# jw007123/hp-Adaptive-Signed-Distance-Field-Octree

Measured on AMD Instinct MI355X. Metric: Query() Mpts/sec at targetError=1e-5 (union3 field, 10M SplitMix64 pts per GPU, HBM-resident); Create() ms reported as create_ms, higher is better.
Workload: dtype f64

## Files before the change

hp-adaptive-signed-distance-field-octree_amd/build.py:

```python
import os
import shutil
import subprocess
import sys

HERE = os.path.dirname(os.path.abspath(__file__))
CSRC = os.path.join(HERE, "csrc")
LIBDIR = os.path.join(HERE, "lib")
LIB = os.path.join(LIBDIR, "libhpsdf.so")
HOOKS_LIB = os.path.join(LIBDIR, "libhpsdf_hooks.so")
HOOK_SOURCES = ["frontier.hip", "capi.cpp"]
INCLUDE = os.path.normpath(os.path.join(HERE, "..", "include"))

SOURCES = ["fit_mesh.hip", "fit_analytic.hip", "fit_samples.hip", "fit.hip", "kernels.hip", "mesh_field.hip", "frontier.hip", "fit_mfma.hip", "fit_low.hip", "mesh_build.hip", "cg.hip", "continuity_asm.hip", "surface.hip", "surface_sparse.hip", "query_gradient.hip", "project.hip", "tables.cpp", "builder.cpp", "mesh.cpp", "obj.cpp", "continuity.cpp", "host_query.cpp", "capi.cpp"]
HEADERS = sorted(f for f in os.listdir(CSRC) if f.endswith(".hpp"))
QUERY_SOURCES = ("kernels.hip",)
MESH_SOURCES = ("mesh_field.hip", "fit_mesh.hip")
SOURCE_GROUPS = {"query": QUERY_SOURCES, "mesh": MESH_SOURCES}
PUBLIC_HEADERS = ["hpsdf.h", "hpsdf_octree.hpp"]

FLAGS = ["-O3", "-std=c++17", "-fPIC", "-ffp-contract=off", "-fno-fast-math", "--offload-arch=gfx950",
         "-fvisibility=hidden", "-Wall", "-Wno-unused-function", "-I", INCLUDE]
FLAGS += os.environ.get("HPSDF_EXTRA_FLAGS", "").split()
FILE_FLAGS = {"fit_mfma.hip": ["-mllvm", "-amdgpu-mfma-vgpr-form=1"]}


def hipcc():
    for c in (os.environ.get("HIPCC"), "/opt/rocm/bin/hipcc", shutil.which("hipcc")):
        if c and os.path.exists(c):
            return c
    raise RuntimeError("hipcc not found: the HIP extension cannot be built (there is no CPU fallback)")


def stale():
    if not os.path.exists(LIB) or not os.path.exists(HOOKS_LIB):
        return True
    t = os.path.getmtime(LIB)
    deps = [os.path.join(CSRC, s) for s in SOURCES + HEADERS] + [os.path.join(INCLUDE, h) for h in PUBLIC_HEADERS]
    deps.append(os.path.abspath(__file__))
    return any(os.path.exists(d) and os.path.getmtime(d) > t for d in deps)


def build(force=False, verbose=False):
    if not force and not stale():
        return LIB
    os.makedirs(LIBDIR, exist_ok=True)
    objs = []
    cc = hipcc()
    objdir = os.path.join(HERE, "build")
    os.makedirs(objdir, exist_ok=True)
    procs = []
    for s in SOURCES:
        src = os.path.join(CSRC, s)
        obj = os.path.join(objdir, s + ".o")
        objs.append(obj)
        if (not force and os.path.exists(obj) and os.path.getmtime(obj) > os.path.getmtime(src)
                and all(os.path.getmtime(obj) > os.path.getmtime(os.path.join(CSRC, h)) for h in HEADERS)
                and all(os.path.getmtime(obj) > os.path.getmtime(os.path.join(INCLUDE, h)) for h in PUBLIC_HEADERS)):
            continue
        cmd = [cc] + FLAGS + FILE_FLAGS.get(s, []) + ["-c", src, "-o", obj]
        if verbose:
            print(" ".join(cmd))
        procs.append((s, subprocess.Popen(cmd, stdout=subprocess.PIPE, stderr=subprocess.STDOUT, text=True)))
    for s, p in procs:
        out, _ = p.communicate()
        if p.returncode != 0:
            raise RuntimeError("hipcc failed on %s:\n%s" % (s, out))
        if verbose and out.strip():
            print(out)
    cmd = [cc, "-shared", "-fPIC", "--offload-arch=gfx950", "-o", LIB] + objs
    r = subprocess.run(cmd, stdout=subprocess.PIPE, stderr=subprocess.STDOUT, text=True)
    if r.returncode != 0:
        raise RuntimeError("link failed:\n" + r.stdout)
    build_hooks(cc, objs, verbose)
    return LIB


def build_hooks(cc, objs, verbose=False):
    hookdir = os.path.join(HERE, "build", "hooks")
    os.makedirs(hookdir, exist_ok=True)
    procs, swapped = [], list(objs)
    for s in HOOK_SOURCES:
        obj = os.path.join(hookdir, s + ".o")
        swapped[SOURCES.index(s)] = obj
        cmd = [cc] + FLAGS + ["-DHPSDF_TEST_HOOKS"] + FILE_FLAGS.get(s, []) + ["-c", os.path.join(CSRC, s), "-o", obj]
        if verbose:
            print(" ".join(cmd))
        procs.append((s, subprocess.Popen(cmd, stdout=subprocess.PIPE, stderr=subprocess.STDOUT, text=True)))
    for s, p in procs:
        out, _ = p.communicate()
        if p.returncode != 0:
            raise RuntimeError("hipcc failed on %s (hooks):\n%s" % (s, out))
    r = subprocess.run([cc, "-shared", "-fPIC", "--offload-arch=gfx950", "-o", HOOKS_LIB] + swapped, stdout=subprocess.PIPE,
                       stderr=subprocess.STDOUT, text=True)
    if r.returncode != 0:
        raise RuntimeError("link failed (hooks):\n" + r.stdout)
    return HOOKS_LIB


LAB_LIB = os.path.join(LIBDIR, "libhpsdf_lab.so")


def build_variant(name, flags, sources=QUERY_SOURCES, verbose=False):
    lib = build()
    cc = hipcc()
    out = os.path.join(LIBDIR, "libhpsdf_%s.so" % name)
    if os.path.exists(out) and os.path.getmtime(out) > os.path.getmtime(lib):
        return out
    vdir = os.path.join(HERE, "build", "variant_" + name)
    os.makedirs(vdir, exist_ok=True)
    objs = [os.path.join(HERE, "build", s + ".o") for s in SOURCES]
    procs = []
    for s in sources:
        obj = os.path.join(vdir, s + ".o")
        objs[SOURCES.index(s)] = obj
        cmd = [cc] + FLAGS + list(flags) + FILE_FLAGS.get(s, []) + ["-c", os.path.join(CSRC, s), "-o", obj]
        if verbose:
            print(" ".join(cmd))
        procs.append((s, subprocess.Popen(cmd, stdout=subprocess.PIPE, stderr=subprocess.STDOUT, text=True)))
    for s, p in procs:
        o, _ = p.communicate()
        if p.returncode != 0:
            raise RuntimeError("hipcc failed on %s (%s):\n%s" % (s, name, o))
    r = subprocess.run([cc, "-shared", "-fPIC", "--offload-arch=gfx950", "-o", out] + objs, stdout=subprocess.PIPE, stderr=subprocess.STDOUT, text=True)
    if r.returncode != 0:
        raise RuntimeError("link failed (%s):\n%s" % (name, r.stdout))
    return out


def build_lab(verbose=False):
    return build_variant("lab", ["-DHPSDF_QUERY_LAB_BUILD"], verbose=verbose)


if __name__ == "__main__":
    print(build(force="--force" in sys.argv, verbose=True))
    if "--lab" in sys.argv:
        print(build_lab(verbose=True))
    for a in sys.argv[1:]:
        if a.startswith("--variant="):
            name, _, rest = a[len("--variant="):].partition(":")
            fl, _, srcs = rest.partition(":")
            print(build_variant(name, [f for f in fl.split(",") if f], SOURCE_GROUPS.get(srcs or "query") or tuple(srcs.split(",")), verbose=True))
```

hp-adaptive-signed-distance-field-octree_amd/csrc/field_eval.hpp:

```cpp
#pragma once
#include <hip/hip_runtime.h>

#include "device_types.hpp"

namespace hpsdf {

template <bool LEFT>
__device__ __forceinline__ double sum3(double a, double b, double c) {
    if constexpr (LEFT) return (a + b) + c;
    else return a + (b + c);
}
template <bool LEFT>
__device__ __forceinline__ double prod3(double a, double b, double c) {
    if constexpr (LEFT) return (a * b) * c;
    else return a * (b * c);
}
__device__ __forceinline__ double sqrtExact(double x) {
    const uint32_t hi = (uint32_t)__double2hiint(x);
    const bool plain = hi - 0x10000000u < 0x7FF00000u - 0x10000000u;
    if (__builtin_amdgcn_ballot_w64(!plain) != 0ull) return sqrt(x);
    const double y = __builtin_amdgcn_rsq(x);
    double g = x * y, h = y * 0.5;
    const double r = __builtin_fma(-h, g, 0.5);
    g = __builtin_fma(g, r, g);
    h = __builtin_fma(h, r, h);
    double d = __builtin_fma(-g, g, x);
    g = __builtin_fma(d, h, g);
    d = __builtin_fma(-g, g, x);
    return __builtin_fma(d, h, g);
}

template <bool LEFT>
__device__ __forceinline__ double norm3(double x, double y, double z) { return sqrtExact(sum3<LEFT>(x * x, y * y, z * z)); }

template <bool LEFT>
__device__ __forceinline__ double primEval(const hpsdf_prim& pr, double x, double y, double z) {
    const double* p = pr.p;
    switch (pr.kind) {
        case HPSDF_PRIM_SPHERE:
            return norm3<LEFT>(x - p[0], y - p[1], z - p[2]) - p[3];
        case HPSDF_PRIM_BOX: {
            const double qx = fabs(x - p[0]) - p[3];
            const double qy = fabs(y - p[1]) - p[4];
            const double qz = fabs(z - p[2]) - p[5];
            const double outside = norm3<LEFT>(fmax(qx, 0.0), fmax(qy, 0.0), fmax(qz, 0.0));
            const double inside = fmin(fmax(qx, fmax(qy, qz)), 0.0);
            return outside + inside;
        }
        case HPSDF_PRIM_TORUS_Y: {
            const double dx = x - p[0], dy = y - p[1], dz = z - p[2];
            const double l = sqrtExact(dx * dx + dz * dz) - p[3];
            return sqrtExact(l * l + dy * dy) - p[4];
        }
        case HPSDF_PRIM_PLANE:
            return (p[0] * x + (p[1] * y + p[2] * z)) + p[3];
        default:
            return 0.0;
    }
}

template <bool LEFT>
__device__ __forceinline__ double analyticEval(const FieldDev& f, double x, double y, double z) {
    double acc = primEval<LEFT>(f.prims[0], x, y, z);
    for (int i = 1; i < f.nPrims; ++i) {
        const double d = primEval<LEFT>(f.prims[i], x, y, z);
        switch (f.prims[i].op) {
            case HPSDF_OP_UNION: acc = fmin(acc, d); break;
            case HPSDF_OP_INTERSECT: acc = fmax(acc, d); break;
            default: acc = fmax(acc, -d); break;
        }
    }
    return acc;
}

}
```

hp-adaptive-signed-distance-field-octree_amd/csrc/fit_kernels.hpp:

```cpp
#pragma once
#include <hip/hip_runtime.h>

#include <cstdint>

#include "device_types.hpp"
#include "field_glue.hpp"
#include "launch.hpp"

namespace hpsdf {


constexpr int kFitPiece = 8;
#ifndef HPSDF_FIT_MIN_WAVES
#define HPSDF_FIT_MIN_WAVES 4
#endif

__device__ __forceinline__ double fitRowAny(double acc, double a1, const double* __restrict__ tk, double n2,
                                            const double* __restrict__ F, int nq) {
    int k = 0;
    for (; k + 4 <= nq; k += 4) {
        const double f0 = F[k], f1 = F[k + 1], f2 = F[k + 2], f3 = F[k + 3];
        const double t0 = tk[k], t1 = tk[k + 1], t2 = tk[k + 2], t3 = tk[k + 3];
        acc = acc + (a1 * t0 * n2) * f0;
        acc = acc + (a1 * t1 * n2) * f1;
        acc = acc + (a1 * t2 * n2) * f2;
        acc = acc + (a1 * t3 * n2) * f3;
    }
    for (; k < nq; ++k) acc = acc + (a1 * tk[k] * n2) * F[k];
    return acc;
}

template <int KIND, bool CSG, int DEG, int R, bool LEFT>
__device__ __forceinline__ void fitBlockBody(const FitBlock blk, const FitTask* __restrict__ tasks, double* __restrict__ arena,
                                             double* __restrict__ errs, double* __restrict__ mirror,
                                             const DeviceTables* __restrict__ T, const FieldDev& field, const RootMap& rm, double* lds) {
    static_assert(R == 1 || DEG > 0, "cell blocking needs a compile-time degree");
    __shared__ double sNl[13 * 11];
    __shared__ double sRec[26];
    __shared__ int32_t sMeshStack[kFitThreads / 64][kMeshStack];
    __shared__ unsigned char sPosI[KIND == kFieldMesh ? 64 : 4], sPosJK[KIND == kFieldMesh ? 64 : 4];
    const int tid = threadIdx.x;
    const int deg = DEG > 0 ? DEG : (int)blk.degree;
    const int nq = 4 * deg + 1, nq2 = nq * nq, G = blk.nTasks;
    const int rowStart = blk.rowStart, rowEnd = blk.rowEnd, nrows = rowEnd - rowStart;
    const int gl = nq * (nq - 1) / 2;
    const int planes = blk.planesPerChunk;
    const int depth = blk.depth;
    const bool split = blk.split != 0;

    double* sT = lds;
    double* sR = sT + (deg + 1) * nq;
    double* sW = sR + nq;
    double* sC = sW + nq;
    double* sF = sC + 8 * G;

    stageQueryTables(T, sNl, sRec);
    for (int q = tid; q < nq; q += kFitThreads) {
        const double x = T->roots[gl + q];
        sR[q] = x;
        sW[q] = T->weights[gl + q];
        double m2 = 0.0, m1 = 1.0;
        sT[q] = 1.0;
        for (int i = 1; i <= deg; ++i) {
            const double l = T->rec[i][0] * x * m1 - T->rec[i][1] * m2;
            m2 = m1, m1 = l;
            sT[i * nq + q] = l;
        }
    }
    for (int g = tid; g < G; g += kFitThreads) {
        const FitTask& tk = tasks[blk.firstTask + g];
        double sc[3];
        for (int a = 0; a < 3; ++a) {
            sc[a] = (double)(tk.bmax[a] - tk.bmin[a]) * 0.5;
            sC[8 * g + 3 + a] = (double)((tk.bmin[a] + tk.bmax[a]) / 2.0f);
            sC[8 * g + a] = sc[a];
        }
        sC[8 * g + 6] = prod3<LEFT>(sc[0], sc[1], sc[2]);
        sC[8 * g + 7] = __longlong_as_double((long long)tk.sampleOff);
    }
    __syncthreads();

    const bool wide = DEG == 0 && nrows > kFitThreads;
    const int slot = wide ? 0 : tid / nrows;
    const int g2 = slot * R;
    const int r0 = rowStart + (wide ? tid : tid % nrows);
    const int r1 = r0 + kFitThreads;
    const bool act0 = wide ? (r0 < rowEnd) : (tid < ((G + R - 1) / R) * nrows);
    const bool act1 = wide && r1 < rowEnd;
    int i0a = 0, i1a = 0, i2a = 0, i0b = 0, i1b = 0, i2b = 0;
    double n0a = 0, n1a = 0, n2a = 0, n0b = 0, n1b = 0, n2b = 0;
    if (act0) {
        i0a = T->bidx[r0][0], i1a = T->bidx[r0][1], i2a = T->bidx[r0][2];
        n0a = sNl[i0a * 11 + depth], n1a = sNl[i1a * 11 + depth], n2a = sNl[i2a * 11 + depth];
    }
    if (act1) {
        i0b = T->bidx[r1][0], i1b = T->bidx[r1][1], i2b = T->bidx[r1][2];
        n0b = sNl[i0b * 11 + depth], n1b = sNl[i1b * 11 + depth], n2b = sNl[i2b * 11 + depth];
    }
    constexpr int NQF = DEG > 0 ? 4 * DEG + 1 : 1;
    double tkReg[NQF];
    if (DEG > 0) {
#pragma unroll
        for (int k = 0; k < NQF; ++k) tkReg[k] = sT[i2a * nq + k];
    }
    uint32_t meshHint = 0xFFFFFFFFu;
    double acc[R];
#pragma unroll
    for (int r = 0; r < R; ++r) acc[r] = 0.0;
    double acc1 = 0.0;

    const int cellStride = planes * nq2;
    for (int iBase = 0; iBase < nq; iBase += planes) {
        const int np = min(planes, nq - iBase);
        if constexpr (KIND == kFieldMesh) {
            if (tid < nq) {
                int rank = 0;
                for (int b = 0; b < nq; ++b) rank += sR[b] < sR[tid] ? 1 : 0;
                sPosJK[rank] = (unsigned char)tid;
            }
            if (tid >= 64 && tid < 64 + np) {
                const int a = tid - 64;
                int rank = 0;
                for (int b = 0; b < np; ++b) rank += sR[iBase + b] < sR[iBase + a] ? 1 : 0;
                sPosI[rank] = (unsigned char)a;
            }
            __syncthreads();
        }
        if constexpr (KIND != kFieldMesh) {
            const int cols = G * nq2;
            for (int c0 = 0; c0 < cols; c0 += kFitThreads) {
                const int cc = c0 + tid;
                const bool activeS = cc < cols;
                const int ccl = activeS ? cc : cols - 1;
                const int g = ccl / nq2, jk = ccl - g * nq2, j = jk / nq, k = jk - j * nq;
                const double* c = sC + 8 * g;
                const double uy = sR[j] * c[1] + c[4], uz = sR[k] * c[2] + c[5];
                const double wy = uy * rm.bounds[1] + rm.centre[1];
                const double wz = uz * rm.bounds[2] + rm.centre[2];
                const double wj = sW[j], wk = sW[k], c6 = c[6];
                const uint64_t sbase = (uint64_t)__double_as_longlong(c[7]) + (uint64_t)(j * nq + k);
                for (int il = 0; il < np; ++il) {
                    const int i = iBase + il;
                    const double ux = sR[i] * c[0] + c[3];
                    const double wx = ux * rm.bounds[0] + rm.centre[0];
                    const uint64_t sidx = sbase + (uint64_t)(i * nq2);
                    const double fv = activeS ? fieldEvalWorld<KIND, CSG, LEFT>(field, wx, wy, wz, sidx, sNl, sRec, meshHint) : 0.0;
                    if (activeS) {
                        sF[g * cellStride + il * nq2 + jk] = c6 * prod3<LEFT>(sW[i], wj, wk) * fv;
                        if (split) const_cast<double*>(field.samples)[sidx] = fv;
                    }
                }
            }
        } else {
            const int chunkSamples = np * nq2, total = G * chunkSamples;
            const float invChunk = 1.0f / (float)chunkSamples;
            for (int s0 = 0; s0 < total; s0 += kFitThreads) {
                const int s = s0 + tid;
                const bool activeS = s < total;
                const int sc = activeS ? s : total - 1;
                int g = (int)(((float)sc + 0.5f) * invChunk);
                int rem = sc - g * chunkSamples;
                if (rem < 0) {
                    --g;
                    rem += chunkSamples;
                } else if (rem >= chunkSamples) {
                    ++g;
                    rem -= chunkSamples;
                }
                if constexpr (KIND == kFieldMesh) rem = meshSampleOrder(rem, np, nq, sPosI, sPosJK);
                const double* c = sC + 8 * g;
                const int il = rem / nq2, jk = rem - il * nq2, j = jk / nq, k = jk - j * nq, i = iBase + il;
                const double ux = sR[i] * c[0] + c[3], uy = sR[j] * c[1] + c[4], uz = sR[k] * c[2] + c[5];
                const double wx = ux * rm.bounds[0] + rm.centre[0];
                const double wy = uy * rm.bounds[1] + rm.centre[1];
                const double wz = uz * rm.bounds[2] + rm.centre[2];
                const uint64_t sidx = (uint64_t)__double_as_longlong(c[7]) + (uint64_t)((i * nq + j) * nq + k);
                double fv;
                if constexpr (KIND == kFieldMesh) {
                    const double mv = (double)meshSignedDistanceWave(field.mesh, V3{(float)wx, (float)wy, (float)wz}, activeS, meshHint,
                                                                     sMeshStack[tid >> 6]);
                    fv = activeS ? applyCsg<CSG>(field, mv, wx, wy, wz, sNl, sRec) : 0.0;
                } else {
                    fv = activeS ? fieldEvalWorld<KIND, CSG, LEFT>(field, wx, wy, wz, sidx, sNl, sRec, meshHint) : 0.0;
                }
                if (activeS) {
                    sF[g * cellStride + rem] = c[6] * prod3<LEFT>(sW[i], sW[j], sW[k]) * fv;
                    if constexpr (KIND != kFieldMesh)
                        if (split) const_cast<double*>(field.samples)[sidx] = fv;
                }
            }
        }
        __syncthreads();
        if (act0) {
            const double* tj = sT + i1a * nq;
            const double* tk = sT + i2a * nq;
            for (int il = 0; il < np; ++il) {
                const double* F = sF + g2 * cellStride + il * nq2;
                const double a0 = sT[i0a * nq + iBase + il] * n0a;
#ifdef HPSDF_FIT_ROW_UNROLL
#pragma unroll HPSDF_FIT_ROW_UNROLL
#endif
                for (int j = 0; j < nq; ++j) {
                    const double a1 = a0 * tj[j] * n1a;
                    if constexpr (DEG > 0 && DEG <= 5) {
                        double lp[NQF];
#pragma unroll
                        for (int k = 0; k < NQF; ++k) lp[k] = a1 * tkReg[k] * n2a;
#pragma unroll
                        for (int r = 0; r < R; ++r) {
                            const double* Fr = F + r * cellStride + j * nq;
                            double f[NQF];
#pragma unroll
                            for (int k = 0; k < NQF; ++k) f[k] = Fr[k];
#pragma unroll
                            for (int k = 0; k < NQF; ++k) acc[r] = acc[r] + lp[k] * f[k];
                        }
                    } else if constexpr (DEG > 5) {
                        const double* Fr = F + j * nq;
#pragma unroll
                        for (int k0 = 0; k0 < NQF; k0 += kFitPiece) {
                            double lp[kFitPiece], f[kFitPiece];
#pragma unroll
                            for (int k = 0; k < kFitPiece; ++k)
                                if (k0 + k < NQF) f[k] = Fr[k0 + k];
#pragma unroll
                            for (int k = 0; k < kFitPiece; ++k)
                                if (k0 + k < NQF) lp[k] = a1 * tkReg[k0 + k] * n2a;
#pragma unroll
                            for (int k = 0; k < kFitPiece; ++k)
                                if (k0 + k < NQF) acc[0] = acc[0] + lp[k] * f[k];
                        }
                    } else {
                        acc[0] = fitRowAny(acc[0], a1, tk, n2a, F + j * nq, nq);
                    }
                }
            }
        }
        if (act1) {
            const double* tj = sT + i1b * nq;
            const double* tk = sT + i2b * nq;
            for (int il = 0; il < np; ++il) {
                const double* F = sF + il * nq2;
                const double a0 = sT[i0b * nq + iBase + il] * n0b;
                for (int j = 0; j < nq; ++j) {
                    const double a1 = a0 * tj[j] * n1b;
                    acc1 = fitRowAny(acc1, a1, tk, n2b, F + j * nq, nq);
                }
            }
        }
        __syncthreads();
    }

    const bool weighted = blk.weighted != 0;
    const int stashStride = weighted ? rowEnd : nrows, stashBase = weighted ? 0 : rowStart;
    const int outBase = split ? 0 : stashBase;
    if (act0) {
#pragma unroll
        for (int r = 0; r < R; ++r)
            if (g2 + r < G) {
                const uint64_t at = tasks[blk.firstTask + g2 + r].outOff + (r0 - outBase);
                arena[at] = acc[r];
                if (mirror != nullptr) mirror[at] = acc[r];
                sF[(g2 + r) * stashStride + (r0 - stashBase)] = acc[r];
            }
    }
    if (act1) {
        arena[tasks[blk.firstTask].outOff + (r1 - outBase)] = acc1;
        sF[r1 - stashBase] = acc1;
    }
    if (weighted && rowStart > 0) {
        for (int s = tid; s < G * rowStart; s += kFitThreads) {
            const int g = s / rowStart, r = s - g * rowStart;
            const FitTask& tk = tasks[blk.firstTask + g];
            const double v = arena[tk.copyOff + r];
            arena[tk.outOff + r] = v;
            sF[g * stashStride + r] = v;
        }
    }
    __syncthreads();
    for (int g = tid; g < G; g += kFitThreads) {
        const int first = deg > 0 ? (int)T->count[deg - 1] : 0;
        double e = 0.0;
        for (int r = first > rowStart ? first : rowStart; r < rowEnd; ++r)
            if (T->bidx[r][3] == deg) {
                const double c = sF[g * stashStride + (r - stashBase)];
                e = e + c * c;
            }
        errs[tasks[blk.firstTask + g].errSlot] = e;
    }
}

template <int KIND, bool CSG, bool LEFT>
__global__ __launch_bounds__(kFitThreads, HPSDF_FIT_MIN_WAVES) void fit_multi_kernel(const FitBlock* __restrict__ blocks,
                                                                const FitTask* __restrict__ tasks, double* __restrict__ arena,
                                                                double* __restrict__ errs, const DeviceTables* __restrict__ T,
                                                                FieldDev field, RootMap rm, const uint32_t* __restrict__ count,
                                                                uint32_t countValue) {
    extern __shared__ double lds[];
    const uint32_t n = count ? *count : countValue;
    if (blockIdx.x >= n) return;
    const FitBlock blk = blocks[n - 1u - blockIdx.x];
    switch (blk.degree) {
        case 2: fitBlockBody<KIND, CSG, 2, 1, LEFT>(blk, tasks, arena, errs, nullptr, T, field, rm, lds); break;
        case 3: fitBlockBody<KIND, CSG, 3, 1, LEFT>(blk, tasks, arena, errs, nullptr, T, field, rm, lds); break;
        case 4: fitBlockBody<KIND, CSG, 4, 1, LEFT>(blk, tasks, arena, errs, nullptr, T, field, rm, lds); break;
        case 5: fitBlockBody<KIND, CSG, 5, 1, LEFT>(blk, tasks, arena, errs, nullptr, T, field, rm, lds); break;
        case 6: fitBlockBody<KIND, CSG, 6, 1, LEFT>(blk, tasks, arena, errs, nullptr, T, field, rm, lds); break;
        case 7: fitBlockBody<KIND, CSG, 7, 1, LEFT>(blk, tasks, arena, errs, nullptr, T, field, rm, lds); break;
        case 8: fitBlockBody<KIND, CSG, 8, 1, LEFT>(blk, tasks, arena, errs, nullptr, T, field, rm, lds); break;
        default: fitBlockBody<KIND, CSG, 0, 1, LEFT>(blk, tasks, arena, errs, nullptr, T, field, rm, lds); break;
    }
}

template <int KIND, bool CSG, int DEG, int R, bool LEFT>
__global__ __launch_bounds__(kFitThreads, HPSDF_FIT_MIN_WAVES) void fit_kernel(const FitBlock* __restrict__ blocks,
                                                          const FitTask* __restrict__ tasks, double* __restrict__ arena,
                                                          double* __restrict__ errs, double* __restrict__ mirror,
                                                          const DeviceTables* __restrict__ T, FieldDev field, RootMap rm,
                                                          const uint32_t* __restrict__ range) {
    extern __shared__ double lds[];
    uint32_t b = blockIdx.x;
    if (range != nullptr) {
        if (b >= range[1]) return;
        b += range[0];
    }
    fitBlockBody<KIND, CSG, DEG, R, LEFT>(blocks[b], tasks, arena, errs, mirror, T, field, rm, lds);
}

template <int KIND, bool CSG, bool LEFT>
__global__ __launch_bounds__(256) void field_kernel(FieldDev f, const DeviceTables* __restrict__ T,
                                                    const double* __restrict__ xyz, size_t n, double* __restrict__ out) {
    __shared__ double sNl[13 * 11];
    __shared__ double sRec[26];
    stageQueryTables(T, sNl, sRec);
    __syncthreads();
    const size_t stride = (size_t)gridDim.x * blockDim.x;
    uint32_t hint = 0xFFFFFFFFu;
    for (size_t i = (size_t)blockIdx.x * blockDim.x + threadIdx.x; i < n; i += stride)
        out[i] = fieldEvalWorld<KIND, CSG, LEFT>(f, xyz[3 * i], xyz[3 * i + 1], xyz[3 * i + 2], i, sNl, sRec, hint);
}

template <int KIND, bool CSG, bool LEFT>
static void launchFitT(hipStream_t stream, int degree, int cellsPerThread, const FitBlock* dBlocks, uint32_t nBlocks,
                       size_t ldsBytes, const FitTask* dTasks, double* dArena, double* dErrs, double* dMeans,
                       const DeviceTables* dTables, const FieldDev& field, const RootMap& rm, const uint32_t* dRange) {
#define HPSDF_FIT_LAUNCH(D, RR)                                                                                       \
    hipLaunchKernelGGL((fit_kernel<KIND, CSG, D, RR, LEFT>), dim3(nBlocks), dim3(kFitThreads), ldsBytes, stream, dBlocks, \
                       dTasks, dArena, dErrs, dMeans, dTables, field, rm, dRange)
#define HPSDF_FIT_CASE(D)       \
    case D:                     \
        HPSDF_FIT_LAUNCH(D, 1); \
        break;
    if (cellsPerThread != 1 && cellsPerThread != 4) cellsPerThread = 1;
    switch (degree) {
        HPSDF_FIT_CASE(2)
        HPSDF_FIT_CASE(3)
        HPSDF_FIT_CASE(4)
        HPSDF_FIT_CASE(5)
        HPSDF_FIT_CASE(6)
        HPSDF_FIT_CASE(7)
        HPSDF_FIT_CASE(8)
        default:
            HPSDF_FIT_LAUNCH(0, 1);
    }
#undef HPSDF_FIT_CASE
#undef HPSDF_FIT_LAUNCH
}

template <int KIND, bool CSG, bool LEFT>
static void launchFitMultiT(hipStream_t stream, const FitBlock* dBlocks, uint32_t maxBlocks, size_t ldsBytes, const FitTask* dTasks,
                            double* dArena, double* dErrs, const DeviceTables* dTables, const FieldDev& field, const RootMap& rm,
                            const uint32_t* dCount) {
    hipLaunchKernelGGL((fit_multi_kernel<KIND, CSG, LEFT>), dim3(maxBlocks), dim3(kFitThreads), ldsBytes, stream, dBlocks, dTasks, dArena, dErrs,
                       dTables, field, rm, dCount, maxBlocks);
}

template <int KIND, bool CSG, bool LEFT>
static void launchFieldT(hipStream_t stream, const FieldDev& f, const DeviceTables* dTables, const double* dXyz,
                         size_t n, double* dOut) {
    hipLaunchKernelGGL((field_kernel<KIND, CSG, LEFT>), dim3(gridFor(n)), dim3(256), 0, stream, f, dTables, dXyz, n, dOut);
}

#define HPSDF_DISPATCH_FIELD_ORDER(FN, K, C, field, ...)  \
    do {                                                  \
        if ((field).leftAssoc) FN<K, C, true>(__VA_ARGS__); \
        else FN<K, C, false>(__VA_ARGS__);                \
    } while (0)
#define HPSDF_DISPATCH_FIELD(FN, K, field, ...)                                                  \
    do {                                                                                         \
        if ((field).csgOp >= 0) HPSDF_DISPATCH_FIELD_ORDER(FN, K, true, field, __VA_ARGS__);     \
        else HPSDF_DISPATCH_FIELD_ORDER(FN, K, false, field, __VA_ARGS__);                       \
    } while (0)

template <int KIND>
void launchFitKind(hipStream_t stream, int degree, int cellsPerThread, const FitBlock* dBlocks, uint32_t nBlocks, size_t ldsBytes,
                   const FitTask* dTasks, double* dArena, double* dErrs, double* dMirror, const DeviceTables* dTables,
                   const FieldDev& field, const RootMap& rm, const uint32_t* dRange) {
    HPSDF_DISPATCH_FIELD(launchFitT, KIND, field, stream, degree, cellsPerThread, dBlocks, nBlocks, ldsBytes, dTasks, dArena,
                         dErrs, dMirror, dTables, field, rm, dRange);
}
template <int KIND>
void launchFitMultiKind(hipStream_t stream, const FitBlock* dBlocks, uint32_t maxBlocks, size_t ldsBytes, const FitTask* dTasks,
                        double* dArena, double* dErrs, const DeviceTables* dTables, const FieldDev& field, const RootMap& rm,
                        const uint32_t* dCount) {
    HPSDF_DISPATCH_FIELD(launchFitMultiT, KIND, field, stream, dBlocks, maxBlocks, ldsBytes, dTasks, dArena, dErrs, dTables, field, rm, dCount);
}
template <int KIND>
void launchFieldKind(hipStream_t stream, const FieldDev& f, const DeviceTables* dTables, const double* dXyz, size_t n, double* dOut) {
    HPSDF_DISPATCH_FIELD(launchFieldT, KIND, f, stream, f, dTables, dXyz, n, dOut);
}
#undef HPSDF_DISPATCH_FIELD
#undef HPSDF_DISPATCH_FIELD_ORDER

#define HPSDF_FIT_KIND_UNIT(EXTERN, K)                                                                                                 \
    EXTERN template void launchFitKind<K>(hipStream_t, int, int, const FitBlock*, uint32_t, size_t, const FitTask*, double*, double*, \
                                          double*, const DeviceTables*, const FieldDev&, const RootMap&, const uint32_t*);            \
    EXTERN template void launchFitMultiKind<K>(hipStream_t, const FitBlock*, uint32_t, size_t, const FitTask*, double*, double*,      \
                                               const DeviceTables*, const FieldDev&, const RootMap&, const uint32_t*);                \
    EXTERN template void launchFieldKind<K>(hipStream_t, const FieldDev&, const DeviceTables*, const double*, size_t, double*);
HPSDF_FIT_KIND_UNIT(extern, kFieldAnalytic)
HPSDF_FIT_KIND_UNIT(extern, kFieldSamples)
HPSDF_FIT_KIND_UNIT(extern, kFieldMesh)

}
```

Before: 93610.

## Batch analytic field evaluation across x-lines in the fit kernel

Adds a line evaluator for analytic primitives that evaluates N x-points sharing the same y,z at once. The y/z terms and the primitive loads are hoisted out of the per-point loop and reused across the N points. The fit kernel uses it for analytic fields with a per-degree piece size, and reloads the tk register table after the field stage to ease register pressure during evaluation. A compiler flag is also added for fit_analytic.hip. This targets the Create() fit cost, not Query(), and the extra per-thread arrays may raise VGPR use.

After: 93550 (median of 3 runs). Within noise of the previous version (-0.1%).

```diff
diff --git a/hp-adaptive-signed-distance-field-octree_amd/build.py b/hp-adaptive-signed-distance-field-octree_amd/build.py
--- a/hp-adaptive-signed-distance-field-octree_amd/build.py
+++ b/hp-adaptive-signed-distance-field-octree_amd/build.py
@@ -21,7 +21,8 @@
 FLAGS = ["-O3", "-std=c++17", "-fPIC", "-ffp-contract=off", "-fno-fast-math", "--offload-arch=gfx950",
          "-fvisibility=hidden", "-Wall", "-Wno-unused-function", "-I", INCLUDE]
 FLAGS += os.environ.get("HPSDF_EXTRA_FLAGS", "").split()
-FILE_FLAGS = {"fit_mfma.hip": ["-mllvm", "-amdgpu-mfma-vgpr-form=1"]}
+FILE_FLAGS = {"fit_mfma.hip": ["-mllvm", "-amdgpu-mfma-vgpr-form=1"],
+              "fit_analytic.hip": ["-mllvm", "-instcombine-max-copied-from-constant-users=100000"]}
 
 
 def hipcc():
diff --git a/hp-adaptive-signed-distance-field-octree_amd/csrc/field_eval.hpp b/hp-adaptive-signed-distance-field-octree_amd/csrc/field_eval.hpp
--- a/hp-adaptive-signed-distance-field-octree_amd/csrc/field_eval.hpp
+++ b/hp-adaptive-signed-distance-field-octree_amd/csrc/field_eval.hpp
@@ -73,4 +73,84 @@
     return acc;
 }
 
+template <bool LEFT, int N>
+__device__ __forceinline__ void analyticEvalLine(const FieldDev& f, const double (&x)[N], double y, double z, double (&acc)[N]) {
+    for (int i = 0; i < f.nPrims; ++i) {
+        const hpsdf_prim& pr = f.prims[i];
+        double d[N];
+        switch (pr.kind) {
+            case HPSDF_PRIM_SPHERE: {
+                const double p0 = pr.p[0], p3 = pr.p[3];
+                const double dy = y - pr.p[1], dz = z - pr.p[2];
+                const double yy = dy * dy, zz = dz * dz, yz = yy + zz;
+#pragma unroll
+                for (int il = 0; il < N; ++il) {
+                    const double dx = x[il] - p0, xx = dx * dx;
+                    d[il] = sqrtExact(LEFT ? (xx + yy) + zz : xx + yz) - p3;
+                }
+                break;
+            }
+            case HPSDF_PRIM_BOX: {
+                const double p0 = pr.p[0], p3 = pr.p[3];
+                const double qy = fabs(y - pr.p[1]) - pr.p[4];
+                const double qz = fabs(z - pr.p[2]) - pr.p[5];
+                const double my = fmax(qy, 0.0), mz = fmax(qz, 0.0);
+                const double yy = my * my, zz = mz * mz, yz = yy + zz;
+                const double qyz = fmax(qy, qz);
+#pragma unroll
+                for (int il = 0; il < N; ++il) {
+                    const double qx = fabs(x[il] - p0) - p3;
+                    const double mx = fmax(qx, 0.0), xx = mx * mx;
+                    const double outside = sqrtExact(LEFT ? (xx + yy) + zz : xx + yz);
+                    const double inside = fmin(fmax(qx, qyz), 0.0);
+                    d[il] = outside + inside;
+                }
+                break;
+            }
+            case HPSDF_PRIM_TORUS_Y: {
+                const double p0 = pr.p[0], p3 = pr.p[3], p4 = pr.p[4];
+                const double dy = y - pr.p[1], dz = z - pr.p[2];
+                const double yy = dy * dy, zz = dz * dz;
+#pragma unroll
+                for (int il = 0; il < N; ++il) {
+                    const double dx = x[il] - p0;
+                    const double l = sqrtExact(dx * dx + zz) - p3;
+                    d[il] = sqrtExact(l * l + yy) - p4;
+                }
+                break;
+            }
+            case HPSDF_PRIM_PLANE: {
+                const double p0 = pr.p[0], p3 = pr.p[3];
+                const double yz = pr.p[1] * y + pr.p[2] * z;
+#pragma unroll
+                for (int il = 0; il < N; ++il) d[il] = (p0 * x[il] + yz) + p3;
+                break;
+            }
+            default:
+#pragma unroll
+                for (int il = 0; il < N; ++il) d[il] = 0.0;
+                break;
+        }
+        if (i == 0) {
+#pragma unroll
+            for (int il = 0; il < N; ++il) acc[il] = d[il];
+            continue;
+        }
+        switch (pr.op) {
+            case HPSDF_OP_UNION:
+#pragma unroll
+                for (int il = 0; il < N; ++il) acc[il] = fmin(acc[il], d[il]);
+                break;
+            case HPSDF_OP_INTERSECT:
+#pragma unroll
+                for (int il = 0; il < N; ++il) acc[il] = fmax(acc[il], d[il]);
+                break;
+            default:
+#pragma unroll
+                for (int il = 0; il < N; ++il) acc[il] = fmax(acc[il], -d[il]);
+                break;
+        }
+    }
 }
+
+}
diff --git a/hp-adaptive-signed-distance-field-octree_amd/csrc/fit_kernels.hpp b/hp-adaptive-signed-distance-field-octree_amd/csrc/fit_kernels.hpp
--- a/hp-adaptive-signed-distance-field-octree_amd/csrc/fit_kernels.hpp
+++ b/hp-adaptive-signed-distance-field-octree_amd/csrc/fit_kernels.hpp
@@ -11,6 +11,8 @@
 
 
 constexpr int kFitPiece = 8;
+template <int DEG>
+constexpr int kFieldPiece = DEG == 2 ? 3 : DEG >= 3 && DEG <= 5 ? 4 : 2;
 #ifndef HPSDF_FIT_MIN_WAVES
 #define HPSDF_FIT_MIN_WAVES 4
 #endif
@@ -28,6 +30,25 @@
     }
     for (; k < nq; ++k) acc = acc + (a1 * tk[k] * n2) * F[k];
     return acc;
+}
+
+template <bool CSG, bool LEFT, int N>
+__device__ __forceinline__ void fitFieldPiece(const FieldDev& field, const RootMap& rm, const double* r, const double* w, const double* c,
+                                              double wy, double wz, double wj, double wk, double* F, int nq2, uint64_t s0, bool split,
+                                              const double* sNl, const double* sRec) {
+    double wx[N], fv[N];
+#pragma unroll
+    for (int il = 0; il < N; ++il) {
+        const double ux = r[il] * c[0] + c[3];
+        wx[il] = ux * rm.bounds[0] + rm.centre[0];
+    }
+    analyticEvalLine<LEFT, N>(field, wx, wy, wz, fv);
+#pragma unroll
+    for (int il = 0; il < N; ++il) {
+        const double v = applyCsg<CSG>(field, fv[il], wx[il], wy, wz, sNl, sRec);
+        F[il * nq2] = c[6] * prod3<LEFT>(w[il], wj, wk) * v;
+        if (split) const_cast<double*>(field.samples)[s0 + (uint64_t)(il * nq2)] = v;
+    }
 }
 
 template <int KIND, bool CSG, int DEG, int R, bool LEFT>
@@ -99,7 +120,8 @@
     }
     constexpr int NQF = DEG > 0 ? 4 * DEG + 1 : 1;
     double tkReg[NQF];
-    if (DEG > 0) {
+    constexpr bool kRowPerChunk = KIND == kFieldAnalytic && DEG > 0;
+    if (DEG > 0 && !kRowPerChunk) {
 #pragma unroll
         for (int k = 0; k < NQF; ++k) tkReg[k] = sT[i2a * nq + k];
     }
@@ -126,7 +148,32 @@
             }
             __syncthreads();
         }
-        if constexpr (KIND != kFieldMesh) {
+        if constexpr (KIND == kFieldAnalytic) {
+            constexpr int PIECE = kFieldPiece<DEG>;
+            const int cols = G * nq2;
+            for (int c0 = 0; c0 < cols; c0 += kFitThreads) {
+                const int cc = c0 + tid;
+                if (cc < cols) {
+                    const int g = cc / nq2, jk = cc - g * nq2, j = jk / nq, k = jk - j * nq;
+                    const double* c = sC + 8 * g;
+                    const double uy = sR[j] * c[1] + c[4], uz = sR[k] * c[2] + c[5];
+                    const double wy = uy * rm.bounds[1] + rm.centre[1];
+                    const double wz = uz * rm.bounds[2] + rm.centre[2];
+                    const double wj = sW[j], wk = sW[k];
+                    const uint64_t sbase = (uint64_t)__double_as_longlong(c[7]) + (uint64_t)(j * nq + k);
+#define HPSDF_FIELD_PIECE(N)                                                                                                  \
+    fitFieldPiece<CSG, LEFT, N>(field, rm, sR + iBase + il0, sW + iBase + il0, c, wy, wz, wj, wk, sF + g * cellStride + il0 * nq2 + jk, \
+                                nq2, sbase + (uint64_t)((iBase + il0) * nq2), split, sNl, sRec)
+                    int il0 = 0;
+                    for (; il0 + PIECE <= np; il0 += PIECE) HPSDF_FIELD_PIECE(PIECE);
+                    if constexpr (PIECE > 2)
+                        for (; il0 + 2 <= np; il0 += 2) HPSDF_FIELD_PIECE(2);
+                    if constexpr (PIECE > 1)
+                        if (il0 < np) HPSDF_FIELD_PIECE(1);
+#undef HPSDF_FIELD_PIECE
+                }
+            }
+        } else if constexpr (KIND != kFieldMesh) {
             const int cols = G * nq2;
             for (int c0 = 0; c0 < cols; c0 += kFitThreads) {
                 const int cc = c0 + tid;
@@ -191,6 +238,10 @@
             }
         }
         __syncthreads();
+        if constexpr (kRowPerChunk) {
+#pragma unroll
+            for (int k = 0; k < NQF; ++k) tkReg[k] = sT[i2a * nq + k];
+        }
         if (act0) {
             const double* tj = sT + i1a * nq;
             const double* tk = sT + i2a * nq;
```
